# plurigrid/moose

Measured on AMD Instinct MI355X. Metric: replicated fixed(14,23) matmul elems/sec, higher is better.
Workload: dtype fixed(14,23) over Z_2^128 (exact multi-modular int8-MFMA GEMM)

## Files before the change

csrc/gemm_crt.hip:

```cpp
#include <hip/hip_runtime.h>

#include <algorithm>
#include <cmath>
#include <cstdint>
#include <cstdlib>
#include <cstring>
#include <mutex>

#include "hip_attr.h"
#include "moosex.h"
#include "prf_dev.h"
#include "rss_fused.h"

void mx_ws_note(int dev, int64_t want, bool ok);
bool mx_ws_malloc(void** p, int64_t bytes);
void mx_ws_shared_note(void);

namespace {

using u64 = uint64_t;
using u128 = unsigned __int128;
typedef int v4i __attribute__((ext_vector_type(4)));
typedef int v16i __attribute__((ext_vector_type(16)));

// ... 88 lines not shown
    for (int j = 0; j < n; ++j)
      if (j != i) {
        W *= (u128)kModuli[j];
        rest = (int)((int64_t)rest * kModuli[j] % p);
      }
    const int inv = modinv(rest, p);
    for (int k = 0; k < 8; ++k) t.rc.W[i][k] = (uint16_t)(W >> (16 * k));
    t.rc.rcp[i] = 1.0f / (float)p;
    t.ep.p[i] = p;
    t.ep.pf[i] = (float)p;
    t.ep.rcp[i] = 1.0f / (float)p;
    t.ep.t16[i] = (int)((1 << 16) % p);
    t.pa.p[i] = t.pb.p[i] = p;
    t.pa.rcp[i] = t.pb.rcp[i] = 1.0f / (float)p;
    int pw = 1 % p;
    for (int j = 0; j < nbytes; ++j) {
      const int wb = pw, wa = (int)((int64_t)pw * inv % p);
      t.pb.w[i][j / 4] |= (uint32_t)wb << (8 * (j % 4));
      t.pa.w[i][j / 4] |= (uint32_t)wa << (8 * (j % 4));
      pw = pw * 256 % p;
    }
    const int negb = (p - pw) % p;
    t.pb.neg[i] = (uint32_t)negb;
    t.pa.neg[i] = (uint32_t)((int64_t)negb * inv % p);
    if (i == 0) {
      t.pa.mul0 = (uint32_t)inv;
      t.pb.mul0 = 1;
    }
  }
  for (int k = 0; k < 8; ++k) t.rc.Mw[k] = (uint16_t)(Mw >> (16 * k));
  std::memset(&t.r4, 0, sizeof t.r4);
  t.r4.groups = (n + 3) / 4;
  for (int i = 0; i < n; ++i) {
    u128 W = 0;
    for (int k = 0; k < 8; ++k) W |= (u128)t.rc.W[i][k] << (16 * k);
    int carry = 0;
    for (int d = 0; d < nbytes; ++d) {
      int b = (int)((W >> (8 * d)) & 0xff) + carry;
      carry = b >= 128;
      b -= 256 * carry;
      t.r4.wd[i / 4][d] |= (uint32_t)(uint8_t)(int8_t)b << (8 * (i % 4));
    }
    int R = (int)std::lround(16777216.0 / kModuli[i]);
    for (int d = 0; d < 3; ++d) {
      int b = (R & 0xff);
      R >>= 8;
      if (b >= 128) {
        b -= 256;
        R += 1;
      }
      t.r4.rd[i / 4][d] |= (uint32_t)(uint8_t)(int8_t)b << (8 * (i % 4));
    }
  }
  (void)wbits;
}

const Tables& tables_for(int words, int n) {
  static std::mutex mu;
  static Tables cache[3][kMaxMod + 1];
  std::lock_guard<std::mutex> lk(mu);
  Tables& t = cache[words][n];
  if (t.n != n || t.words != words) build_tables(words, n, t);
  return t;
}

__device__ __forceinline__ uint32_t pack4(int a, int b, int c, int d) {
  const uint32_t lo = __builtin_amdgcn_perm((uint32_t)b, (uint32_t)a, 0x0c0c0400u);
  const uint32_t hi = __builtin_amdgcn_perm((uint32_t)d, (uint32_t)c, 0x0c0c0400u);
  return __builtin_amdgcn_perm(hi, lo, 0x05040100u);
}

template <class T>
struct Words;
template <>
struct Words<u64> {
  static constexpr int N = 2;
};
template <>
struct Words<u128> {
  static constexpr int N = 4;
};

template <int NW>
__device__ __forceinline__ int residue(const uint32_t (&x)[NW], const uint32_t (&w)[4],
                                       uint32_t neg, float p, float rcp) {
  uint32_t s = (x[NW - 1] >> 31) * neg;
#pragma unroll
  for (int q = 0; q < NW; ++q) s = __builtin_amdgcn_udot4(x[q], w[q], s, false);
  const float fs = (float)s;
  const float qt = __builtin_rintf(fs * rcp);
  return (int)__builtin_fmaf(-qt, p, fs);
}

typedef float f2 __attribute__((ext_vector_type(2)));
template <int NW>
__device__ __forceinline__ void residue2(const uint32_t (&xa)[NW], const uint32_t (&xb)[NW],
                                         const uint32_t (&w)[4], uint32_t neg, float p,
                                         float rcp, int& ra, int& rb) {
  uint32_t sa = 0, sb = 0;
#pragma unroll
  for (int q = 0; q < NW; ++q) {
    sa = __builtin_amdgcn_udot4(xa[q], w[q], sa, false);
    sb = __builtin_amdgcn_udot4(xb[q], w[q], sb, false);
  }
  const f2 sg = {(float)(xa[NW - 1] >> 31), (float)(xb[NW - 1] >> 31)};
  const float nf = (float)neg;
  const f2 fs = __builtin_elementwise_fma(sg, (f2){nf, nf}, (f2){(float)sa, (float)sb});
  f2 qt = fs * (f2){rcp, rcp};
  qt.x = __builtin_rintf(qt.x);
  qt.y = __builtin_rintf(qt.y);
  const f2 r = __builtin_elementwise_fma(-qt, (f2){p, p}, fs);
  ra = (int)r.x;
  rb = (int)r.y;
}

struct PrepSrcs {
  int n = 0;
  int mode[6];
  const void* x0[6];
  const void* x1[6];
  int64_t dual[6];
};

template <class T, bool TRANS, int ROWS, bool PK = true>
__global__ void __launch_bounds__(256)
    k_crt_prep(const T* __restrict__ X0, const T* __restrict__ X1, int64_t R, int64_t K,
               int64_t xs, int mode_all, int8_t* __restrict__ out, int64_t tiles, int64_t nkb,
               int64_t nkb_s, const PrepTab tab, const PrepSrcs src) {
  constexpr int NW = Words<T>::N;
  const int64_t total = tiles * nkb * (ROWS * 4);
  const int64_t b = blockIdx.y;
  const int mode = src.n > 0 ? src.mode[b] : mode_all;
  const T* x0 = src.n > 0 ? (const T*)src.x0[b] : X0 + b * xs;
  const T* x1 = src.n > 0 ? (const T*)src.x1[b] : (mode ? X1 + b * xs : x0);
  const int n = tab.n;
  const int64_t plane = tiles * nkb_s * (int64_t)(ROWS * BK);
  int8_t* ob = out + b * n * plane;
  for (int64_t g = blockIdx.x * (int64_t)blockDim.x + threadIdx.x; g < total;
       g += (int64_t)gridDim.x * blockDim.x) {
    const int c = (int)(g & 3);
    const int r = (int)((g >> 2) & (ROWS - 1));
    const int64_t q = g / (ROWS * 4);
    const int64_t kb = q % nkb, t = q / nkb;
    const int64_t row = t * ROWS + r;
    const int64_t k0 = kb * BK + c * 16;
    uint32_t v[16][NW];
#pragma unroll
    for (int j = 0; j < 16; ++j) {
      const int64_t k = k0 + j;
      T e = 0;
      if (row < R) {
        if (!TRANS) {
          if (k < K) e = mode == 2 ? (T)(x0[row * K + k] + x1[row * K + k]) : x0[row * K + k];
          else if (mode == 1 && k < 2 * K) e = x1[row * K + (k - K)];
        } else {
          if (k < K)
            e = (mode & 1) ? (T)(x0[k * R + row] + x1[k * R + row]) : x0[k * R + row];
          else if (mode == 1 && k < 2 * K) e = x0[(k - K) * R + row];
          else if (mode == 2 && k < 2 * K) e = x1[(k - K) * R + row];
        }
      }
#pragma unroll
      for (int w = 0; w < NW; ++w) v[j][w] = (uint32_t)(e >> (32 * w));
    }
    const int64_t boff = (t * nkb_s + kb) * (int64_t)(ROWS * BK) + img_off(r, c);
    auto emit = [&](int8_t* base) __attribute__((always_inline)) {
    {
      int rr[16];
#pragma unroll
      for (int j = 0; j < 16; ++j) rr[j] = (int)(v[j][0] * tab.mul0);
      v4i o;
#pragma unroll
      for (int u = 0; u < 4; ++u) o[u] = (int)pack4(rr[4 * u], rr[4 * u + 1], rr[4 * u + 2], rr[4 * u + 3]);
      *(v4i*)base = o;
    }
    for (int i = 1; i < n; ++i) {
      const uint32_t w[4] = {tab.w[i][0], tab.w[i][1], tab.w[i][2], tab.w[i][3]};
      const uint32_t neg = tab.neg[i];
      const float p = (float)tab.p[i], rcp = tab.rcp[i];
      int rr[16];
      if constexpr (PK) {
#pragma unroll
        for (int j = 0; j < 16; j += 2)
          residue2<NW>(v[j], v[j + 1], w, neg, p, rcp, rr[j], rr[j + 1]);
      } else {
#pragma unroll
        for (int j = 0; j < 16; ++j) rr[j] = residue<NW>(v[j], w, neg, p, rcp);
      }
      v4i o;
#pragma unroll
      for (int u = 0; u < 4; ++u) o[u] = (int)pack4(rr[4 * u], rr[4 * u + 1], rr[4 * u + 2], rr[4 * u + 3]);
      *(v4i*)(base + i * plane) = o;
    }
    };
    emit(ob + boff);
    if (src.n > 0 && src.dual[b]) {
#pragma unroll
      for (int j = 0; j < 16; ++j) {
        const int64_t k = k0 + j;
        if (row < R && k < K) {
          T e = 0;
#pragma unroll
          for (int w = 0; w < NW; ++w) e |= (T)v[j][w] << (32 * w);
          e += TRANS ? x1[k * R + row] : x1[row * K + k];
#pragma unroll
          for (int w = 0; w < NW; ++w) v[j][w] = (uint32_t)(e >> (32 * w));
        }
      }
      emit(ob + src.dual[b] + boff);
    }
  }
}

struct ShareSrc {
  const void* x = nullptr;
  int kind = 0;
  int frac = 0;
  int j0 = 0;
  uint64_t nonce = 0;
  mxd::KeySrc key;
};
struct SrcPlan {
  const void* x;
  int kind, pad;
  double scale;
  uint64_t nonce;
  int ph[4];
  int64_t off[4];
};

template <bool TRANS, int ROWS, bool PK>
__global__ void __launch_bounds__(256)
    k_crt_prep_src(const SrcPlan s, const mxd::KeySrc keys, int64_t R, int64_t K,
                   int8_t* __restrict__ out, int64_t tiles, int64_t nkb, const PrepTab tab) {
  using T = u128;
  constexpr int NW = 4;
  __shared__ uint32_t rks[1][mxd::kKeyWords];
  __shared__ uint4 xch[4][4][64];
  mxd::stage_keys(rks, keys, 1);
  const int lane = threadIdx.x & 63;
  const int p = lane & 3;
  uint4(*xw)[64] = xch[threadIdx.x >> 6];
  const int n = tab.n;
  const int64_t plane = tiles * nkb * (int64_t)(ROWS * BK);
  const int64_t total = tiles * ROWS * nkb * 4;
  for (int64_t g = blockIdx.x * (int64_t)blockDim.x + threadIdx.x; g < total;
       g += (int64_t)gridDim.x * blockDim.x) {
    const int c = (int)((g >> 2) & 3);
    const int rlow = (int)((g >> 4) & 3);
    const int64_t rest = g >> 6;
    int64_t row, kb, i0, istep;
    if (!TRANS) {
      const int64_t q = rest / (ROWS / 4);
      kb = 4 * (q % (nkb / 4)) + p;
      row = (q / (nkb / 4)) * ROWS + (rest % (ROWS / 4)) * 4 + rlow;
      i0 = row * K + (kb - p) * BK + c * 16;
      istep = 1;
    } else {
      const int64_t q = rest >> 4;
      kb = q % nkb;
      row = (q / nkb) * 256 + 64 * p + (rest & 15) * 4 + rlow;
      i0 = (kb * BK + c * 16) * R + (row - 64 * p);
      istep = R;
    }
    const bool live = row < R;
    const int64_t t = row / ROWS;
    const int r = (int)(row % ROWS);
    uint32_t v[16][NW];
#pragma unroll
    for (int jj = 0; jj < 4; ++jj) {
      uint32_t w[16];
      mx::chacha_block(rks[0], s.nonce, mx::ks_block_of((uint64_t)(i0 + (4 * jj + p) * istep)), w);
#pragma unroll
      for (int q = 0; q < 4; ++q)
        xw[q][lane ^ q] = make_uint4(w[4 * q], w[4 * q + 1], w[4 * q + 2], w[4 * q + 3]);
      __builtin_amdgcn_fence(__ATOMIC_RELEASE, "wavefront");
      __builtin_amdgcn_wave_barrier();
      __builtin_amdgcn_fence(__ATOMIC_ACQUIRE, "wavefront");
#pragma unroll
      for (int u = 0; u < 4; ++u) {
        const uint4 e = xw[p][((lane & ~3) | u) ^ p];
        v[4 * jj + u][0] = live ? e.x : 0u;
        v[4 * jj + u][1] = live ? e.y : 0u;
        v[4 * jj + u][2] = live ? e.z : 0u;
        v[4 * jj + u][3] = live ? e.w : 0u;
      }
      __builtin_amdgcn_fence(__ATOMIC_RELEASE, "wavefront");
      __builtin_amdgcn_wave_barrier();
      __builtin_amdgcn_fence(__ATOMIC_ACQUIRE, "wavefront");
    }
    const int64_t boff = (t * nkb + kb) * (int64_t)(ROWS * BK) + img_off(r, c);
    auto emit = [&](int8_t* base) __attribute__((always_inline)) {
      {
        int rr[16];
#pragma unroll
        for (int j = 0; j < 16; ++j) rr[j] = (int)(v[j][0] * tab.mul0);
        v4i o;
#pragma unroll
        for (int u = 0; u < 4; ++u) o[u] = (int)pack4(rr[4 * u], rr[4 * u + 1], rr[4 * u + 2], rr[4 * u + 3]);
        *(v4i*)base = o;
      }
      for (int i = 1; i < n; ++i) {
        const uint32_t w[4] = {tab.w[i][0], tab.w[i][1], tab.w[i][2], tab.w[i][3]};
        const uint32_t neg = tab.neg[i];
        const float pf = (float)tab.p[i], rcp = tab.rcp[i];
        int rr[16];
        if constexpr (PK) {
#pragma unroll
          for (int j = 0; j < 16; j += 2)
            residue2<NW>(v[j], v[j + 1], w, neg, pf, rcp, rr[j], rr[j + 1]);
        } else {
#pragma unroll
          for (int j = 0; j < 16; ++j) rr[j] = residue<NW>(v[j], w, neg, pf, rcp);
        }
        v4i o;
#pragma unroll
        for (int u = 0; u < 4; ++u) o[u] = (int)pack4(rr[4 * u], rr[4 * u + 1], rr[4 * u + 2], rr[4 * u + 3]);
        *(v4i*)(base + i * plane) = o;
      }
    };
    auto step = [&](bool sum) __attribute__((always_inline)) {
#pragma unroll
      for (int j = 0; j < 16; ++j) {
        T h = 0;
#pragma unroll
        for (int w = 0; w < NW; ++w) h |= (T)v[j][w] << (32 * w);
        const T x = live ? mxf::share_plain<T>(s.kind, s.x, i0 + 64 * p + j * istep, s.scale) : (T)0;
        const T other = mxf::share_masked<T>(s.kind, x, h);
        h = sum ? (T)(h + other) : other;
#pragma unroll
        for (int w = 0; w < NW; ++w) v[j][w] = (uint32_t)(h >> (32 * w));
      }
    };
#pragma nounroll
    for (int ph = 0; ph < 4; ++ph) {
      if (s.ph[0] != ph && s.ph[1] != ph && s.ph[2] != ph && s.ph[3] != ph) continue;
      if (ph == 1) step(false);
      if (ph == 2) step(true);
      if (ph == 3) {
#pragma unroll
        for (int j = 0; j < 16; ++j)
#pragma unroll
          for (int w = 0; w < NW; ++w) v[j][w] = 0;
      }
#pragma nounroll
      for (int e = 0; e < 4; ++e)
        if (s.ph[e] == ph) emit(out + s.off[e] + boff);
    }
  }
}

template <class T>
__global__ void __launch_bounds__(256)
    k_add_pair(const T* __restrict__ a, const T* __restrict__ b, T* __restrict__ o, int64_t n) {
  for (int64_t i = blockIdx.x * (int64_t)blockDim.x + threadIdx.x; i < n;
       i += (int64_t)gridDim.x * blockDim.x)
    o[i] = a[i] + b[i];
}

__device__ inline int64_t xcd_remap(int64_t bid, int64_t nwg) {
  const int64_t q = nwg / 8, r = nwg % 8;
  const int64_t x = bid % 8;
  return (x < r ? x * (q + 1) : r * (q + 1) + (x - r) * q) + bid / 8;
}

constexpr int waitcnt_vm_lgkm0(int vm) { return (vm & 15) | ((vm >> 4) << 14) | (7 << 4); }

__device__ __forceinline__ int centered_mod(int acc, float pf, float rcp, int t16) {
  const int hi = acc >> 16, lo = acc & 0xffff;
  const int s = __mul24(hi, t16) + lo;
  const float fs = (float)s;
  const float qt = __builtin_rintf(fs * rcp);
  return (int)__builtin_fmaf(-qt, pf, fs);
}

template <int WR, int WC, int BN, int MINW>
__global__ void __launch_bounds__(64 * WR * WC, MINW)
    k_crt_gemm(const int8_t* __restrict__ RA, const int8_t* __restrict__ RB,
               int8_t* __restrict__ CR, int tiles_m, int tiles_n, int nkb, int gM,
               const EpiTab ep, int dma_mask, int bcast) {
  constexpr int NW = WR * WC;
  constexpr int MI = BM / WR / 32, NJ = BN / WC / 32;
  constexpr int kImgB = BN * BK;
  constexpr int kStageBytes = kImg + kImgB;
  constexpr int NPIECE = kStageBytes / 1024;
  constexpr int PPW = NPIECE / NW;
  static_assert(PPW * NW == NPIECE, "stage pieces must split evenly over the waves");
  extern __shared__ __attribute__((aligned(16))) int8_t smem[];
  const int ntiles = tiles_m * tiles_n;
  const int tid_flat = (int)xcd_remap(blockIdx.x, ntiles);
  const int group = tid_flat / (gM * tiles_n);
  const int first_m = group * gM;
  const int gm = tiles_m - first_m < gM ? tiles_m - first_m : gM;
  const int in_group = tid_flat % (gM * tiles_n);
  const int tm = first_m + in_group % gm, tn = in_group / gm;
  const int g = blockIdx.y;
  const int mi = g % ep.n;
  const int8_t* ga = RA + ((int64_t)((bcast & 1) ? mi : g) * tiles_m + tm) * nkb * (int64_t)kImg;
  const int8_t* gb = RB + ((int64_t)((bcast & 2) ? mi : g) * tiles_n + tn) * nkb * (int64_t)kImgB;

  const int lane = threadIdx.x & 63;
  const int wave = __builtin_amdgcn_readfirstlane(threadIdx.x >> 6);
  const int wr = wave / WC, wc = wave % WC;
  const int half = lane >> 5;
  const int sw = swz(lane >> 2);
  const int rowa = (wr * (BM / WR) + (lane & 31)) * BK;
  const int rowb = kImg + (wc * (BN / WC) + (lane & 31)) * BK;
  const int co0 = 16 * (half ^ sw), co1 = 16 * ((2 + half) ^ sw);

  const int8_t* srcs[PPW];
  int dsts[PPW], steps[PPW];
#pragma unroll
  for (int t = 0; t < PPW; ++t) {
    const int pc = wave + NW * t;
    const bool is_b = pc >= 16;
    const int pp = is_b ? pc - 16 : pc;
    srcs[t] = (is_b ? gb : ga) + pp * 1024 + lane * 16;
    dsts[t] = (is_b ? kImg : 0) + pp * 1024;
    steps[t] = is_b ? kImgB : kImg;
  }
  auto dma = [&](int kb, int t, int8_t* dst_stage) {
    if (!((dma_mask >> (wave + NW * t >= 16 ? 1 : 0)) & 1)) return;
    __builtin_amdgcn_global_load_lds((const void*)(srcs[t] + (int64_t)kb * steps[t]),
                                     (__attribute__((address_space(3))) void*)(dst_stage + dsts[t]),
                                     16, 0, 0);
  };

  v16i acc[MI][NJ];
#pragma unroll
  for (int i = 0; i < MI; ++i)
// ... 939 lines not shown
  launch_recon<T>(p, tb, 3, M, N, cr, C, 0, st);
  const hipError_t e = hipGetLastError();
  return e != hipSuccess ? -100 - (int)e : 0;
}

}

extern "C" {

int mx_gemm_asym(int words, int64_t M, int64_t N, int64_t K, const void* S0, const void* S1,
                 const void* T0, const void* T1, int rolled, void* C, void* stream) {
  if (M == 0 || N == 0) return 0;
  if (!rolled && (!S1 || !T1)) return -2;
  hipStream_t st = (hipStream_t)stream;
  if (words == 1)
    return run_crt_asym<u64>(M, N, K, (const u64*)S0, (const u64*)S1, (const u64*)T0,
                             (const u64*)T1, rolled, (u64*)C, st);
  if (words == 2)
    return run_crt_asym<u128>(M, N, K, (const u128*)S0, (const u128*)S1, (const u128*)T0,
                              (const u128*)T1, rolled, (u128*)C, st);
  return -2;
}

int mx_gemm_asym_src(int words, int64_t M, int64_t N, int64_t K, const void* S0, const void* T0,
                     const int64_t* xsrc, const int64_t* ysrc, void* C, void* stream) {
  if (M == 0 || N == 0) return 0;
  if (words != 2) return -7;
  if ((!xsrc && !S0) || (!ysrc && !T0)) return -2;
  ShareSrc sx, sy;
  auto fill = [](ShareSrc& s, const int64_t* a) {
    s.x = (const void*)(intptr_t)a[0];
    s.kind = (int)a[1];
    s.frac = (int)a[2];
    s.j0 = (int)a[3];
    const uint32_t* slot[1] = {(const uint32_t*)(intptr_t)a[4]};
    s.key = mxd::keysrc_slots(slot, 1);
    s.nonce = (uint64_t)a[5];
  };
  if (xsrc) fill(sx, xsrc);
  if (ysrc) fill(sy, ysrc);
  if ((xsrc && !sx.key.slot[0]) || (ysrc && !sy.key.slot[0])) return -2;
  return run_crt_asym<u128>(M, N, K, (const u128*)S0, nullptr, (const u128*)T0, nullptr, 1,
                            (u128*)C, (hipStream_t)stream, xsrc ? &sx : nullptr,
                            ysrc ? &sy : nullptr);
}

int mx_crt_moduli(int words, int64_t kprime) {
  if (words != 1 && words != 2) return -2;
  return moduli_needed(words, kprime);
}

int mx_crt_tables(int words, int n, int32_t* p_out, uint8_t* wa_out, uint8_t* wb_out,
                  int32_t* nega_out, int32_t* negb_out, uint16_t* W_out, uint16_t* Mw_out) {
  if ((words != 1 && words != 2) || n < 1 || n > kMaxMod) return -2;
  const Tables& t = tables_for(words, n);
  for (int i = 0; i < n; ++i) {
    p_out[i] = t.ep.p[i];
    for (int j = 0; j < 16; ++j) {
      wa_out[i * 16 + j] = (uint8_t)(t.pa.w[i][j / 4] >> (8 * (j % 4)));
      wb_out[i * 16 + j] = (uint8_t)(t.pb.w[i][j / 4] >> (8 * (j % 4)));
    }
    nega_out[i] = (int32_t)t.pa.neg[i];
    negb_out[i] = (int32_t)t.pb.neg[i];
    if (i == 0) {
      nega_out[0] = (int32_t)t.pa.mul0;
      negb_out[0] = 1;
    }
    for (int k = 0; k < 8; ++k) W_out[i * 8 + k] = t.rc.W[i][k];
  }
  for (int k = 0; k < 8; ++k) Mw_out[k] = t.rc.Mw[k];
  return 0;
}

int mx_crt_tables4(int words, int n, uint32_t* wd_out, uint32_t* rd_out) {
  if ((words != 1 && words != 2) || n < 1 || n > kMaxMod) return -2;
  const Tables& t = tables_for(words, n);
  for (int g = 0; g < t.r4.groups; ++g) {
    for (int d = 0; d < 16; ++d) wd_out[g * 16 + d] = t.r4.wd[g][d];
    for (int d = 0; d < 3; ++d) rd_out[g * 3 + d] = t.r4.rd[g][d];
  }
  return t.r4.groups;
}

int mxh_gemm_crt(int words, int64_t batch, int64_t M, int64_t N, int64_t K, const void* A0,
                 const void* A1, const void* B0, const void* B1, int mode, void* C,
                 int accumulate, void* stream) {
  hipStream_t st = (hipStream_t)stream;
  if (words == 1)
    return run_crt<u64>(batch, M, N, K, (const u64*)A0, (const u64*)A1, M * K, (const u64*)B0,
                        (const u64*)B1, K * N, nullptr, mode, (u64*)C, accumulate, st);
  if (words == 2)
    return run_crt<u128>(batch, M, N, K, (const u128*)A0, (const u128*)A1, M * K,
                         (const u128*)B0, (const u128*)B1, K * N, nullptr, mode, (u128*)C,
                         accumulate, st);
  return -2;
}

int mxh_gemm_crt_strided(int words, int64_t batch, int64_t M, int64_t N, int64_t K,
                         const void* A0, const void* A1, int64_t a_bstride, const void* B0,
                         const void* B1, int64_t b_bstride, int mode, void* C, int accumulate,
                         void* stream) {
  hipStream_t st = (hipStream_t)stream;
  if (words == 1)
    return run_crt<u64>(batch, M, N, K, (const u64*)A0, (const u64*)A1, a_bstride,
                        (const u64*)B0, (const u64*)B1, b_bstride, nullptr, mode, (u64*)C,
                        accumulate, st);
  if (words == 2)
    return run_crt<u128>(batch, M, N, K, (const u128*)A0, (const u128*)A1, a_bstride,
                         (const u128*)B0, (const u128*)B1, b_bstride, nullptr, mode, (u128*)C,
                         accumulate, st);
  return -2;
}

int mxh_crt_roll(int words, int64_t batch, int64_t M, int64_t N, int64_t K, const void* A0,
                 int64_t a_bstride, int64_t roll, const void* B0, const void* B1, const void* rb,
                 void* C, int accumulate, void* stream) {
  hipStream_t st = (hipStream_t)stream;
  const int64_t bs = K * N;
  if (words == 1)
    return run_crt<u64>(batch, M, N, K, (const u64*)A0, nullptr, a_bstride, (const u64*)B0,
                        (const u64*)B1, bs, (const int8_t*)rb, 1, (u64*)C, accumulate, st, roll);
  if (words == 2)
    return run_crt<u128>(batch, M, N, K, (const u128*)A0, nullptr, a_bstride, (const u128*)B0,
                         (const u128*)B1, bs, (const int8_t*)rb, 1, (u128*)C, accumulate, st,
                         roll);
  return -2;
}

int64_t mxh_crt_b_bytes(int words, int64_t batch, int64_t N, int64_t K, int mode) {
  if (words != 1 && words != 2) return 0;
  const CPlan p = make_cplan(words, batch, BM, N, K, mode);
  return p.n < 0 ? 0 : p.rb_bytes;
}

int mxh_crt_prep_b(int words, int64_t batch, int64_t K, int64_t N, const void* B0,
                   const void* B1, int mode, void* rb, void* stream) {
  const CPlan p = make_cplan(words, batch, BM, N, K, mode);
  if (p.n < 0) return -6;
  const Tables& tb = tables_for(words, p.n);
  hipStream_t st = (hipStream_t)stream;
  if (words == 1)
    launch_prep<u64>(p, tb, true, batch, N, K, K * N, (const u64*)B0, (const u64*)B1, mode,
                     (int8_t*)rb, st);
  else if (words == 2)
    launch_prep<u128>(p, tb, true, batch, N, K, K * N, (const u128*)B0, (const u128*)B1, mode,
                      (int8_t*)rb, st);
  else
    return -2;
  const hipError_t e = hipGetLastError();
  return e != hipSuccess ? -100 - (int)e : 0;
}

int mxh_crt_with_b(int words, int64_t batch, int64_t M, int64_t N, int64_t K, const void* A0,
                   const void* A1, int64_t a_bstride, int mode, const void* rb, void* C,
                   int accumulate, void* stream) {
  hipStream_t st = (hipStream_t)stream;
  if (words == 1)
    return run_crt<u64>(batch, M, N, K, (const u64*)A0, (const u64*)A1, a_bstride, nullptr,
                        nullptr, 0, (const int8_t*)rb, mode, (u64*)C, accumulate, st);
  if (words == 2)
    return run_crt<u128>(batch, M, N, K, (const u128*)A0, (const u128*)A1, a_bstride, nullptr,
                         nullptr, 0, (const int8_t*)rb, mode, (u128*)C, accumulate, st);
  return -2;
}

}
// ... 1 lines not shown
```

csrc/moosex.h:

```cpp
#pragma once
#include <stdint.h>

#ifdef __cplusplus
extern "C" {
#endif

enum mx_binop { MX_ADD = 0, MX_SUB = 1, MX_MUL = 2, MX_AND = 3, MX_OR = 4, MX_XOR = 5 };
enum mx_unop { MX_NEG = 0, MX_NOT = 1, MX_SHL = 2, MX_SHR = 3, MX_SAR = 4 };
enum mx_cmpop { MX_LT = 0, MX_GT = 1, MX_EQ = 2, MX_MSB = 3 };
enum mx_cross { MX_CROSS_ARITH = 0, MX_CROSS_BOOL = 1 };
enum mx_share_src { MX_SHARE_F64 = 2, MX_SHARE_MIRROR = 8 };

typedef struct {
  uint32_t rk[44];
} mx_aes_key;

int mx_version(void);
int mx_device_count(void);

int mx_ew_binary(int dev, int op, int words, const void* a, int64_t na, const void* b,
                 int64_t nb, void* out, int64_t n, void* stream);
int mx_ew_binary_slot(int dev, int op, int words, const void* a, const void* b, int64_t nb,
                      void* out, int64_t m, int nparties, int which, void* stream);
int mx_add_zs3(int dev, int words, const void* v, const void* r, void* out0, void* out1,
// ... 19 lines not shown
              int64_t w_slot_stride, int64_t N, int64_t C, int64_t H, int64_t W, int64_t mult,
              int64_t KH, int64_t KW, int64_t sh, int64_t sw, int64_t pt, int64_t pl,
              int64_t dh, int64_t dw, int64_t OH, int64_t OW, int nhwc, void* stream);
int mx_ew_binary_slot2(int dev, int op, int words, const void* a0, const void* a1,
                       const void* b, int64_t nb, void* out0, void* out1, int64_t m,
                       int nparties, int which0, int which1, void* stream);
int mx_mul_trunc3_kv(int dev, int words, const void* x0, const void* x1, const void* y0,
                     const void* y1, void* out0, void* out1, int64_t n, int64_t ostride,
                     const uint32_t* slots, uint64_t nmul, int m, const uint64_t* nonces,
                     const int64_t* views, void* stream);
int mx_mul_trunc3_open(int dev, int words, const void* x, int64_t xstride, double* out,
                       int64_t n, const uint32_t* slots, uint64_t nmul, int m,
                       const uint64_t* nonces, int frac, void* stream);
int mx_ew_add3(int dev, int words, const void* a, const void* b, const void* c, void* out,
               int64_t n, void* stream);
int mx_lincomb2(int dev, int words, int nin, const void* const* ins, const int64_t* coef,
                const void* b, int64_t nb, void* out0, void* out1, int64_t m, int nparties,
                int which0, int which1, void* stream);
int mx_sum_views2(int dev, int words, const void* base0, const void* base1, int64_t is0,
                  int64_t is1, int64_t ps0, int64_t ps1, int k, void* out0, void* out1, int64_t m,
                  int nparties, void* stream);
int mx_slot_place2(int dev, int words, const void* x0, const void* x1, void* out0, void* out1,
                   int64_t m, int nparties, int which0, int which1, void* stream);
int mx_ew_compare(int dev, int op, int words, const void* a, int64_t na, const void* b,
                  int64_t nb, uint8_t* out, int64_t n, void* stream);
int mx_bit_extract(int dev, int words, const void* a, uint8_t* out, int64_t n, int bit,
                   void* stream);
int mx_ring_inject(int dev, int words, const uint8_t* bits, void* out, int64_t n, int bit,
                   void* stream);
int mx_encode(int dev, int words, const double* x, void* out, int64_t n, int frac,
              void* stream);
int mx_addn_decode(int dev, int words, const void* a, const void* b, const void* c,
                   const void* d, double* out, int64_t n, int frac, void* stream);
int mx_decode(int dev, int words, const void* x, double* out, int64_t n, int frac,
              void* stream);
int mx_fill(int dev, int words, void* out, int64_t n, uint64_t lo, uint64_t hi, void* stream);
int mx_bit_planes(int dev, int words, const void* a, uint8_t* out, int64_t outer, int64_t inner,
                  int start, int count, void* stream);
int mx_weighted_sum(int dev, int words, const void* a, const void* w, void* out, int64_t outer,
                    int64_t k, int64_t inner, void* stream);
int mx_sum_axis(int dev, int words, const void* a, void* out, int64_t outer, int64_t red,
                int64_t inner, void* stream);
int mx_prg(int dev, const uint8_t* key16, uint64_t nonce, uint64_t ctr0, void* out,
           int64_t nbytes, void* stream);
int mx_derive_seed(const uint8_t* key16, const uint8_t* sync16, uint8_t* out16);
int mx_aes_encrypt_blocks(const uint8_t* key16, const uint8_t* in, uint8_t* out,
                          int64_t nblocks);
int mx_rss_cross(int dev, int kind, int words, const void* x0, const void* x1,
                 const void* y0, const void* y1, void* out, int64_t n, int nparties,
                 const uint8_t* keys16, uint64_t nonce, void* stream);
int mx_zero_share(int dev, int kind, int words, void* out, int64_t n, int nparties,
                  const uint8_t* keys16, uint64_t nonce, void* stream);
int mx_prf_expand(int dev, int words, void* out, int64_t n, int nkeys,
                  const uint8_t* keys16, uint64_t nonce, void* stream);
int mx_gemm(int dev, int words, int64_t batch, int64_t M, int64_t N, int64_t K,
            const void* A0, const void* A1, const void* B0, const void* B1, int mode,
            void* C, int accumulate, void* stream);
int64_t mx_gemm_workspace_bytes(int words, int64_t batch, int64_t M, int64_t N,
                                int64_t K, int mode);
int64_t mx_workspace_failed_bytes(void);
int64_t mx_workspace_held_bytes(void);
int64_t mx_workspace_shared_count(void);
int mx_gemm_ws(int words, int64_t batch, int64_t M, int64_t N, int64_t K, const void* A0,
               const void* A1, const void* B0, const void* B1, int mode, void* C,
               int accumulate, void* workspace, int64_t ws_bytes, void* stream);
int64_t mx_gemm_b_bytes(int words, int64_t batch, int64_t N, int64_t K, int mode);
int mx_gemm_prep_b(int words, int64_t batch, int64_t K, int64_t N, const void* B0,
                   const void* B1, int mode, void* lb, void* stream);
int mx_gemm_with_b(int words, int64_t batch, int64_t M, int64_t N, int64_t K, const void* A0,
                   const void* A1, int64_t a_bstride, int mode, const void* lb, void* C,
                   int accumulate, void* stream);
int mx_crt_tables4(int words, int n, uint32_t* wd_out, uint32_t* rd_out);
int mx_gemm_roll(int words, int64_t batch, int64_t M, int64_t N, int64_t K, const void* A0,
                 int64_t a_bstride, int64_t roll, const void* B0, const void* B1, const void* lb,
                 void* C, int accumulate, void* stream);
int mx_gemm_strided(int words, int64_t batch, int64_t M, int64_t N, int64_t K, const void* A0,
                    const void* A1, int64_t a_bstride, const void* B0, const void* B1,
                    int64_t b_bstride, int mode, void* C, int accumulate, void* stream);
void mx_set_gemm_impl(int impl);
void mx_set_gemm_crt(int mode);
int mx_crt_moduli(int words, int64_t kprime);
int mx_crt_tables(int words, int n, int32_t* p, uint8_t* wa, uint8_t* wb, int32_t* nega,
                  int32_t* negb, uint16_t* W, uint16_t* Mw);

int mx_trunc_pr3(int dev, int words, const void* s0, void* out0, void* out1, int64_t n, int m,
                 const uint8_t* k0, const uint8_t* k2, const uint64_t* nonces, void* stream);
int mx_share3(int dev, int kind, int words, const void* x, void* out0, void* out1, int64_t n,
              int j, const uint8_t* k_next, const uint8_t* k_all, uint64_t n1, uint64_t na,
              void* stream);

#define MX_KEY_SLOT_WORDS 48
void mx_key_slots(const uint8_t* keys16, int n, uint32_t* out);
int mx_rss_cross_k(int dev, int kind, int words, const void* x0, const void* x1,
                   const void* y0, const void* y1, void* out, int64_t n, int nparties,
                   const uint32_t* slots, int nslots, uint64_t nonce, void* stream);
int mx_rss_cross_kp(int dev, int kind, int words, const void* x0, const void* x1,
                    const void* y0, const void* y1, void* out, int64_t n, int nparties,
                    const uint32_t* const* slot_ptrs, uint64_t nonce, void* stream);
int mx_rss_mul3_kv(int dev, int kind, int words, const void* x0, const void* x1, const void* y0,
                   const void* y1, void* out0, void* out1, int64_t n, const uint32_t* slots,
                   uint64_t nonce, const int64_t* views, void* stream);
int mx_rss_mul3_k(int dev, int kind, int words, const void* x0, const void* x1, const void* y0,
                  const void* y1, void* out0, void* out1, int64_t n, const uint32_t* slots,
                  uint64_t nonce, void* stream);
int mx_ks_adder3_k(int dev, int words, const void* g0, const void* g1, const void* p0,
                   const void* p1, void* og0, void* og1, int64_t n, int nlev,
                   const uint32_t* slots, const uint64_t* nonces, void* stream);
int mx_ks_level3_k(int dev, int words, const void* g0, const void* g1, const void* p0,
                   const void* p1, void* og0, void* og1, void* op0, void* op1, int64_t n,
                   int d, int both, const uint32_t* slots, uint64_t nonce, void* stream);
int mx_ks_cross1(int dev, int words, const void* g0, const void* g1, const void* p0,
                 const void* p1, void* z, int64_t n, int d, int both, const uint8_t* keys16,
                 uint64_t nonce, void* stream);
int mx_ks_cross1_s(int dev, int words, const void* g0, const void* g1, const void* p0,
                   const void* p1, void* z, int64_t n, int d, int both,
                   const uint32_t* const* slots, uint64_t nonce, void* stream);
int mx_ks_cross1x_s(int dev, int words, const void* g0, const void* g1, const void* t0,
                    const void* t1, void* go0, void* go1, const void* p0, const void* p1,
                    void* z, int64_t n, int d, int both, const uint32_t* const* slots,
                    uint64_t nonce, void* stream);
int mx_ks_sum2(int dev, int words, const void* p0, const void* p1, const void* g0,
               const void* g1, const void* t0, const void* t1, void* o0, void* o1, int64_t n,
               void* stream);
int mx_prf_expand_k(int dev, int words, void* out, int64_t n, int nkeys, const uint32_t* slots,
                    uint64_t nonce, void* stream);
int mx_trunc_pr3_k(int dev, int words, const void* s0, void* out0, void* out1, int64_t n, int m,
                   const uint32_t* slot_k0, const uint32_t* slot_k2, const uint64_t* nonces,
                   void* stream);
int mx_trunc_pr3_ko(int dev, int words, const void* s0, void* out0, void* out1, int64_t n,
                    int m, const uint32_t* slot_k0, const uint32_t* slot_k2,
                    const uint64_t* nonces, int64_t ostride, void* stream);
int mx_trunc_pr3_kmo(int dev, int words, const void* s0, void* out0, void* out1, int64_t n,
                     int m, const uint32_t* slot_k0, const uint32_t* slot_k2,
                     const uint64_t* nonces, int64_t ostride, const uint64_t* cm, void* stream);
int mx_share3_k(int dev, int kind, int words, const void* x, void* out0, void* out1, int64_t n,
                int j, const uint32_t* slot_next, const uint32_t* slot_all, uint64_t n1,
                uint64_t na, void* stream);
int mx_ring_extend3_k(int dev, const void* s0, void* out0, void* out1, int64_t n,
                      const uint32_t* slot_k0, const uint32_t* slot_k2, const uint64_t* nonces,
                      void* stream);
int64_t mx_ring_extend3_lat_max(void);

int mx_trunc_party_r0(int dev, int words, int64_t n, int m, int ncomp, const int* roles,
                      const void* s0, const void* s1, void* msg, void* msg_rm, void* out0,
                      void* out1, const uint32_t* const* slots, const uint64_t* nonces,
                      void* stream);
int mx_trunc_party_r1(int dev, int words, int64_t n, int m, int ncomp, const int* roles,
                      const void* msg, const void* rmk, const void* rrt, const void* rrm,
                      void* w, void* out0, void* out1, const uint32_t* const* slots,
                      const uint64_t* nonces, void* stream);
int mx_ring_extend_party_r0(int dev, int64_t n, int ncomp, const int* roles, const void* s0,
                            const void* s1, void* msg, void* msg_R, void* msg_M, void* out0,
                            void* out1, const uint32_t* const* slots, const uint64_t* nonces,
                            void* stream);
int mx_ring_extend_party_r1(int dev, int64_t n, int ncomp, const int* roles, const void* msg,
                            const void* rmk, const void* rR, const void* rM, void* w, void* out0,
                            void* out1, const uint32_t* const* slots, const uint64_t* nonces,
                            void* stream);
int mx_share_party(int dev, int kind, int words, int64_t n, int ncomp, const int* rel,
                   const void* x, void* out0, void* out1, const uint32_t* const* slots,
                   uint64_t n1, uint64_t na, void* stream);
int mx_dot_tail_r0(int dev, int words, int64_t n, int m, int ncomp, const int* roles,
                   const void* const* cross, void* const* msg, void* const* msg_rt,
                   void* const* msg_rm, void* const* out0, void* const* out1,
                   const uint32_t* const* slots, const uint64_t* nonces, void* stream);
int mx_dot_tail_r1(int dev, int words, int64_t n, int m, int ncomp, const int* roles,
// ... 40 lines not shown
```

moose_amd/ops/native.py:

```python
from __future__ import annotations

import ctypes
import os
import threading

import torch

from moose_amd import errors
from moose_amd._native import build as _build

_LIB = None
_LOCK = threading.Lock()

c_i64 = ctypes.c_int64
c_int = ctypes.c_int
c_u64 = ctypes.c_uint64
c_vp = ctypes.c_void_p

_SIGS = {
    "mx_version": (c_int, []),
    "mx_device_count": (c_int, []),
    "mx_ew_binary": (c_int, [c_int, c_int, c_int, c_vp, c_i64, c_vp, c_i64, c_vp, c_i64, c_vp]),
    "mx_ew_unary": (c_int, [c_int, c_int, c_int, c_vp, c_vp, c_i64, c_i64, c_vp]),
    "mx_mul_add2": (c_int, [c_int, c_int, c_vp, c_vp, c_vp, c_vp, c_int, c_int, c_vp, c_vp,
# ... 122 lines not shown
        [c_int, c_int, c_vp, c_vp, c_vp, c_vp, c_vp, c_vp, c_i64, c_int, c_vp, c_vp, c_vp],
    ),
    "mxh_ks_adder3_sum": (
        c_int,
        [c_int, c_vp, c_vp, c_vp, c_vp, c_vp, c_vp, c_i64, c_int, c_vp, c_vp, c_vp, c_int],
    ),
    "mx_ks_level3_k": (
        c_int,
        [c_int, c_int, c_vp, c_vp, c_vp, c_vp, c_vp, c_vp, c_vp, c_vp, c_i64, c_int, c_int,
         c_vp, c_u64, c_vp],
    ),
    "mx_rss_cross_kp": (
        c_int,
        [c_int, c_int, c_int, c_vp, c_vp, c_vp, c_vp, c_vp, c_i64, c_int, c_vp, c_u64, c_vp],
    ),
    "mx_rss_mul3_kv": (
        c_int,
        [c_int, c_int, c_int, c_vp, c_vp, c_vp, c_vp, c_vp, c_vp, c_i64, c_vp, c_u64, c_vp, c_vp],
    ),
    "mx_rss_mul3_k": (
        c_int,
        [c_int, c_int, c_int, c_vp, c_vp, c_vp, c_vp, c_vp, c_vp, c_i64, c_vp, c_u64, c_vp],
    ),
    "mx_trunc_pr3_k": (
        c_int, [c_int, c_int, c_vp, c_vp, c_vp, c_i64, c_int, c_vp, c_vp, c_vp, c_vp],
    ),
    "mx_trunc_pr3_ko": (
        c_int, [c_int, c_int, c_vp, c_vp, c_vp, c_i64, c_int, c_vp, c_vp, c_vp, c_i64, c_vp],
    ),
    "mx_trunc_pr3_kmo": (
        c_int, [c_int, c_int, c_vp, c_vp, c_vp, c_i64, c_int, c_vp, c_vp, c_vp, c_i64, c_vp,
                c_vp],
    ),
    "mx_share3_k": (
        c_int,
        [c_int, c_int, c_int, c_vp, c_vp, c_vp, c_i64, c_int, c_vp, c_vp, c_u64, c_u64, c_vp],
    ),
    "mx_ring_extend3_k": (c_int, [c_int, c_vp, c_vp, c_vp, c_i64, c_vp, c_vp, c_vp, c_vp]),
    "mx_ring_extend3_lat_max": (c_i64, []),
    "mx_trunc_party_r0": (
        c_int,
        [c_int, c_int, c_i64, c_int, c_int, c_vp, c_vp, c_vp, c_vp, c_vp, c_vp, c_vp, c_vp,
         c_vp, c_vp],
    ),
    "mx_trunc_party_r1": (
        c_int,
        [c_int, c_int, c_i64, c_int, c_int, c_vp, c_vp, c_vp, c_vp, c_vp, c_vp, c_vp, c_vp,
         c_vp, c_vp, c_vp],
    ),
    "mx_ring_extend_party_r0": (
        c_int,
        [c_int, c_i64, c_int, c_vp, c_vp, c_vp, c_vp, c_vp, c_vp, c_vp, c_vp, c_vp, c_vp, c_vp],
    ),
    "mx_ring_extend_party_r1": (
        c_int,
        [c_int, c_i64, c_int, c_vp, c_vp, c_vp, c_vp, c_vp, c_vp, c_vp, c_vp, c_vp, c_vp, c_vp],
    ),
    "mx_dot_tail_r0": (
        c_int,
        [c_int, c_int, c_i64, c_int, c_int, c_vp, c_vp, c_vp, c_vp, c_vp, c_vp, c_vp, c_vp,
         c_vp, c_vp],
    ),
    "mx_dot_tail_r1": (
        c_int,
        [c_int, c_int, c_i64, c_int, c_int, c_vp, c_vp, c_vp, c_vp, c_vp, c_vp, c_vp, c_vp,
         c_vp, c_vp, c_vp, c_vp],
    ),
    "mx_dot_tail_r2": (c_int, [c_int, c_int, c_i64, c_int, c_vp, c_vp, c_vp, c_vp, c_vp]),
    "mx_share_party": (
        c_int,
        [c_int, c_int, c_int, c_i64, c_int, c_vp, c_vp, c_vp, c_vp, c_vp, c_u64, c_u64, c_vp],
    ),
    "mx_gemm_b_bytes": (c_i64, [c_int, c_i64, c_i64, c_i64, c_int]),
    "mx_gemm_prep_b": (c_int, [c_int, c_i64, c_i64, c_i64, c_vp, c_vp, c_int, c_vp, c_vp]),
    "mx_gemm_with_b": (
        c_int,
        [c_int, c_i64, c_i64, c_i64, c_i64, c_vp, c_vp, c_i64, c_int, c_vp, c_vp, c_int, c_vp],
    ),
    "mx_share3": (
        c_int,
        [c_int, c_int, c_int, c_vp, c_vp, c_vp, c_i64, c_int, c_vp, c_vp, c_u64, c_u64, c_vp],
    ),
    "mx_crt_tables4": (c_int, [c_int, c_int, c_vp, c_vp]),
    "mx_copy_channels": (c_int, [c_vp, c_vp, c_i64, c_int, c_vp]),
    "mx_stream_cumask": (c_int, [c_vp, c_int, c_vp]),
    "mx_stream_destroy": (c_int, [c_vp]),
    "mx_graph_compose": (c_int, [c_int, c_vp, c_vp, c_vp, c_vp, c_vp, c_vp, c_vp, c_vp, c_vp]),
    "mx_graph_compose_merged": (c_int, [c_int, c_vp, c_vp, c_vp, c_vp, c_vp, c_vp, c_vp, c_vp,
                                        c_vp]),
    "mx_graph_dot": (c_int, [c_vp, ctypes.c_char_p, ctypes.c_uint]),
    "mx_graph_launch": (c_int, [c_vp, c_vp]),
    "mx_enable_peer": (c_int, [c_int, c_int]),
    "mx_alloc_uncached": (c_int, [c_int, c_i64, c_vp]),
    "mx_free_uncached": (c_int, [c_int, c_vp]),
    "mx_graph_build_chain": (c_int, [c_int, c_vp, c_vp, c_vp, c_vp, c_vp, c_vp, c_vp, c_vp,
                                     c_vp]),
    "mx_jobs_r0": (c_int, [c_int, c_int, c_int, c_vp, c_vp, c_i64, c_int, c_int, c_int, c_int,
                           c_vp, c_vp, c_vp, c_vp, c_vp, c_vp]),
    "mx_jobs_r0p": (c_int, [c_int, c_int, c_int, c_vp, c_vp, c_i64, c_int, c_int, c_int, c_int,
                            c_vp, c_vp, c_vp, c_vp, c_vp, c_int, c_vp, c_vp, c_vp]),
    "mx_jobs_r1": (c_int, [c_int, c_int, c_int, c_vp, c_vp, c_i64, c_int, c_int, c_vp, c_vp, c_vp,
                           c_vp, c_vp, c_vp, c_vp, c_vp, c_vp]),
    "mx_jobs_r2": (c_int, [c_int, c_int, c_int, c_vp, c_vp, c_i64, c_int, c_vp, c_vp, c_vp]),
    "mx_bits_front": (c_int, [c_int, c_int, c_int, c_i64, c_vp, c_vp, c_vp, c_vp, c_vp, c_vp,
                              c_vp, c_vp, c_vp, c_vp]),
    "mx_wsum_pair": (c_int, [c_int, c_int, c_int, c_int, c_int, c_int, c_int, c_i64, c_i64,
                             c_vp, c_vp, c_vp, c_vp, c_vp, c_vp, c_vp, c_vp, c_vp, c_vp, c_vp,
                             c_vp, c_vp, c_vp]),
    "mx_bits_b2a": (c_int, [c_int, c_int, c_int, c_int, c_i64, c_int, c_int, c_int, c_int,
                            c_vp, c_vp, c_vp,
                            c_vp, c_vp, c_vp, c_vp, c_vp, c_vp, c_vp, c_vp, c_vp]),
    "mx_key_refresh": (c_int, [c_vp, c_int, c_vp, c_vp, c_vp]),
    "mx_copy_async": (c_int, [c_vp, c_vp, ctypes.c_int64, c_vp]),
    "mx_key_refresh_host": (None, [c_vp, c_u64, c_int, c_vp]),
    "mx_copy_many": (c_int, [c_vp, c_int, c_i64, c_vp]),
    "mx_graph_free": (c_int, [c_vp, c_vp]),
    "mx_gemm_asym": (
        c_int, [c_int, c_i64, c_i64, c_i64, c_vp, c_vp, c_vp, c_vp, c_int, c_vp, c_vp],
    ),
    "mx_gemm_asym_src": (
        c_int, [c_int, c_i64, c_i64, c_i64, c_vp, c_vp, c_vp, c_vp, c_vp, c_vp],
    ),
    "mx_gemm_roll": (
        c_int,
        [c_int, c_i64, c_i64, c_i64, c_i64, c_vp, c_i64, c_i64, c_vp, c_vp, c_vp, c_vp, c_int,
         c_vp],
    ),
}


class NativeError(errors.KernelError):
    pass


def lib():
    global _LIB
    if _LIB is not None:
        return _LIB
    with _LOCK:
        if _LIB is not None:
            return _LIB
        if _build.needs_build() and os.environ.get("MOOSEX_NO_BUILD") != "1":
            _build.build()
        path = os.environ.get("MOOSEX_LIB") or str(_build.LIB)
        try:
            handle = ctypes.CDLL(path, mode=ctypes.RTLD_GLOBAL)
        except OSError as e:
            raise NativeError(f"cannot load {path}: {e}") from e
        for name, (res, args) in _SIGS.items():
            fn = getattr(handle, name)
            fn.restype = res
            fn.argtypes = args
        _LIB = handle
        return _LIB


def loaded_path():
    return str(_build.LIB)


def check(rc, what):
    if rc != 0:
        if rc == -4:
            raise NativeError(workspace_error(what, _ws_failed_bytes(), _ws_held_bytes()))
        raise NativeError(f"{what} failed with code {rc}")

# ... 79 lines not shown
```

Before: 1.398 billion.

## Derive sum-share CRT residues from component residues with carry correction

The fused share-and-prep kernel used to walk up to four phases serially. Each phase recomputed a full multi-word residue reduction for every modulus, and each sum phase re-ran the 128-bit add. It now computes the residues of the random share and the masked share once, then derives the residue of their sum by adding the two and applying a carry-count (kappa) correction times the wrap constant. The f64 plaintext loads are batched up front. This saves dot4 reductions and loop overhead but keeps more live registers (rr, v, kf, xp), and a host-side mx_crt_combine test hook is added.

```diff
diff --git a/csrc/gemm_crt.hip b/csrc/gemm_crt.hip
--- a/csrc/gemm_crt.hip
+++ b/csrc/gemm_crt.hip
@@ -194,21 +194,26 @@
 };
 
 template <int NW>
-__device__ __forceinline__ int residue(const uint32_t (&x)[NW], const uint32_t (&w)[4],
-                                       uint32_t neg, float p, float rcp) {
+__device__ __forceinline__ float residue_f(const uint32_t (&x)[NW], const uint32_t (&w)[4],
+                                           uint32_t neg, float p, float rcp) {
   uint32_t s = (x[NW - 1] >> 31) * neg;
 #pragma unroll
   for (int q = 0; q < NW; ++q) s = __builtin_amdgcn_udot4(x[q], w[q], s, false);
   const float fs = (float)s;
   const float qt = __builtin_rintf(fs * rcp);
-  return (int)__builtin_fmaf(-qt, p, fs);
+  return __builtin_fmaf(-qt, p, fs);
+}
+template <int NW>
+__device__ __forceinline__ int residue(const uint32_t (&x)[NW], const uint32_t (&w)[4],
+                                       uint32_t neg, float p, float rcp) {
+  return (int)residue_f<NW>(x, w, neg, p, rcp);
 }
 
 typedef float f2 __attribute__((ext_vector_type(2)));
 template <int NW>
-__device__ __forceinline__ void residue2(const uint32_t (&xa)[NW], const uint32_t (&xb)[NW],
+__device__ __forceinline__ f2 residue2_f(const uint32_t (&xa)[NW], const uint32_t (&xb)[NW],
                                          const uint32_t (&w)[4], uint32_t neg, float p,
-                                         float rcp, int& ra, int& rb) {
+                                         float rcp) {
   uint32_t sa = 0, sb = 0;
 #pragma unroll
   for (int q = 0; q < NW; ++q) {
@@ -221,9 +226,38 @@
   f2 qt = fs * (f2){rcp, rcp};
   qt.x = __builtin_rintf(qt.x);
   qt.y = __builtin_rintf(qt.y);
-  const f2 r = __builtin_elementwise_fma(-qt, (f2){p, p}, fs);
+  return __builtin_elementwise_fma(-qt, (f2){p, p}, fs);
+}
+template <int NW>
+__device__ __forceinline__ void residue2(const uint32_t (&xa)[NW], const uint32_t (&xb)[NW],
+                                         const uint32_t (&w)[4], uint32_t neg, float p,
+                                         float rcp, int& ra, int& rb) {
+  const f2 r = residue2_f<NW>(xa, xb, w, neg, p, rcp);
   ra = (int)r.x;
   rb = (int)r.y;
+}
+
+__host__ __device__ inline int crt_sum_kappa(uint32_t ta, uint32_t tb, uint32_t ts) {
+  const uint32_t carry = ((ta & tb) | ((ta | tb) & ~ts)) >> 31;
+  return (int)(ta >> 31) + (int)(tb >> 31) - (int)carry - (int)(ts >> 31);
+}
+__host__ __device__ inline float crt_combine_f(float ra, float rb, float kappa, float neg,
+                                               float p, float rcp) {
+  const float fs = __builtin_fmaf(kappa, -neg, ra + rb);
+  const float qt = __builtin_rintf(fs * rcp);
+  return __builtin_fmaf(-qt, p, fs);
+}
+__host__ __device__ inline int crt_combine(int ra, int rb, int kappa, uint32_t neg, float p,
+                                           float rcp) {
+  return (int)crt_combine_f((float)ra, (float)rb, (float)kappa, (float)neg, p, rcp);
+}
+__host__ __device__ inline f2 crt_combine2(f2 ra, f2 rb, f2 kappa, float neg, float p,
+                                           float rcp) {
+  const f2 fs = __builtin_elementwise_fma(kappa, (f2){-neg, -neg}, ra + rb);
+  f2 qt = fs * (f2){rcp, rcp};
+  qt.x = __builtin_rintf(qt.x);
+  qt.y = __builtin_rintf(qt.y);
+  return __builtin_elementwise_fma(-qt, (f2){p, p}, fs);
 }
 
 struct PrepSrcs {
@@ -378,7 +412,7 @@
     const bool live = row < R;
     const int64_t t = row / ROWS;
     const int r = (int)(row % ROWS);
-    uint32_t v[16][NW];
+    uint32_t rr[16][NW], v[16][NW];
 #pragma unroll
     for (int jj = 0; jj < 4; ++jj) {
       uint32_t w[16];
@@ -392,72 +426,125 @@
 #pragma unroll
       for (int u = 0; u < 4; ++u) {
         const uint4 e = xw[p][((lane & ~3) | u) ^ p];
-        v[4 * jj + u][0] = live ? e.x : 0u;
-        v[4 * jj + u][1] = live ? e.y : 0u;
-        v[4 * jj + u][2] = live ? e.z : 0u;
-        v[4 * jj + u][3] = live ? e.w : 0u;
+        rr[4 * jj + u][0] = live ? e.x : 0u;
+        rr[4 * jj + u][1] = live ? e.y : 0u;
+        rr[4 * jj + u][2] = live ? e.z : 0u;
+        rr[4 * jj + u][3] = live ? e.w : 0u;
       }
       __builtin_amdgcn_fence(__ATOMIC_RELEASE, "wavefront");
       __builtin_amdgcn_wave_barrier();
       __builtin_amdgcn_fence(__ATOMIC_ACQUIRE, "wavefront");
     }
+    float kf[16];
+    T xp[16];
+    if (s.kind == MX_SHARE_F64) {
+      double d[16];
+#pragma unroll
+      for (int j = 0; j < 16; ++j)
+        d[j] = live ? ((const double*)s.x)[i0 + 64 * p + j * istep] : 0.0;
+#pragma unroll
+      for (int j = 0; j < 16; ++j) xp[j] = mxf::share_plain<T>(MX_SHARE_F64, d, j, s.scale);
+    } else {
+#pragma unroll
+      for (int j = 0; j < 16; ++j)
+        xp[j] = live ? mxf::share_plain<T>(s.kind, s.x, i0 + 64 * p + j * istep, s.scale) : (T)0;
+    }
+#pragma unroll
+    for (int j = 0; j < 16; ++j) {
+      T h = 0;
+#pragma unroll
+      for (int w = 0; w < NW; ++w) h |= (T)rr[j][w] << (32 * w);
+      const T x = xp[j];
+      const T other = mxf::share_masked<T>(s.kind, x, h);
+#pragma unroll
+      for (int w = 0; w < NW; ++w) v[j][w] = (uint32_t)(other >> (32 * w));
+      kf[j] = (float)crt_sum_kappa(rr[j][NW - 1], v[j][NW - 1],
+                                   (uint32_t)((T)(h + other) >> (32 * (NW - 1))));
+    }
     const int64_t boff = (t * nkb + kb) * (int64_t)(ROWS * BK) + img_off(r, c);
-    auto emit = [&](int8_t* base) __attribute__((always_inline)) {
-      {
-        int rr[16];
-#pragma unroll
-        for (int j = 0; j < 16; ++j) rr[j] = (int)(v[j][0] * tab.mul0);
-        v4i o;
-#pragma unroll
-        for (int u = 0; u < 4; ++u) o[u] = (int)pack4(rr[4 * u], rr[4 * u + 1], rr[4 * u + 2], rr[4 * u + 3]);
-        *(v4i*)base = o;
-      }
-      for (int i = 1; i < n; ++i) {
-        const uint32_t w[4] = {tab.w[i][0], tab.w[i][1], tab.w[i][2], tab.w[i][3]};
-        const uint32_t neg = tab.neg[i];
-        const float pf = (float)tab.p[i], rcp = tab.rcp[i];
-        int rr[16];
+    bool has[4];
+#pragma unroll
+    for (int ph = 0; ph < 4; ++ph)
+      has[ph] = s.ph[0] == ph || s.ph[1] == ph || s.ph[2] == ph || s.ph[3] == ph;
+    const bool do_r = has[0] || has[2], do_v = has[1] || has[2];
+    auto put = [&](int ph, int64_t ioff, const v4i o) __attribute__((always_inline)) {
+#pragma unroll
+      for (int e = 0; e < 4; ++e)
+        if (s.ph[e] == ph) *(v4i*)(out + s.off[e] + ioff + boff) = o;
+    };
+    auto pack16 = [](const int (&q)[16]) __attribute__((always_inline)) {
+      v4i o;
+#pragma unroll
+      for (int u = 0; u < 4; ++u) o[u] = (int)pack4(q[4 * u], q[4 * u + 1], q[4 * u + 2], q[4 * u + 3]);
+      return o;
+    };
+    const v4i zero = {0, 0, 0, 0};
+    {
+      int q[16];
+#pragma unroll
+      for (int j = 0; j < 16; ++j) q[j] = (int)(rr[j][0] * tab.mul0);
+      put(0, 0, pack16(q));
+#pragma unroll
+      for (int j = 0; j < 16; ++j) q[j] = (int)(v[j][0] * tab.mul0);
+      put(1, 0, pack16(q));
+#pragma unroll
+      for (int j = 0; j < 16; ++j) q[j] = (int)((rr[j][0] + v[j][0]) * tab.mul0);
+      put(2, 0, pack16(q));
+      put(3, 0, zero);
+    }
+    for (int i = 1; i < n; ++i) {
+      const uint32_t w[4] = {tab.w[i][0], tab.w[i][1], tab.w[i][2], tab.w[i][3]};
+      const uint32_t neg = tab.neg[i];
+      const float pf = (float)tab.p[i], rcp = tab.rcp[i];
+      const int64_t ioff = i * plane;
+      const float nf = (float)neg;
+      auto res4 = [&](const uint32_t (&x)[16][NW], int u, float (&f)[4])
+                      __attribute__((always_inline)) {
         if constexpr (PK) {
 #pragma unroll
-          for (int j = 0; j < 16; j += 2)
-            residue2<NW>(v[j], v[j + 1], w, neg, pf, rcp, rr[j], rr[j + 1]);
+          for (int j = 0; j < 4; j += 2) {
+            const f2 g = residue2_f<NW>(x[4 * u + j], x[4 * u + j + 1], w, neg, pf, rcp);
+            f[j] = g.x;
+            f[j + 1] = g.y;
+          }
         } else {
 #pragma unroll
-          for (int j = 0; j < 16; ++j) rr[j] = residue<NW>(v[j], w, neg, pf, rcp);
+          for (int j = 0; j < 4; ++j) f[j] = residue_f<NW>(x[4 * u + j], w, neg, pf, rcp);
         }
-        v4i o;
-#pragma unroll
-        for (int u = 0; u < 4; ++u) o[u] = (int)pack4(rr[4 * u], rr[4 * u + 1], rr[4 * u + 2], rr[4 * u + 3]);
-        *(v4i*)(base + i * plane) = o;
-      }
-    };
-    auto step = [&](bool sum) __attribute__((always_inline)) {
-#pragma unroll
-      for (int j = 0; j < 16; ++j) {
-        T h = 0;
-#pragma unroll
-        for (int w = 0; w < NW; ++w) h |= (T)v[j][w] << (32 * w);
-        const T x = live ? mxf::share_plain<T>(s.kind, s.x, i0 + 64 * p + j * istep, s.scale) : (T)0;
-        const T other = mxf::share_masked<T>(s.kind, x, h);
-        h = sum ? (T)(h + other) : other;
-#pragma unroll
-        for (int w = 0; w < NW; ++w) v[j][w] = (uint32_t)(h >> (32 * w));
-      }
-    };
-#pragma nounroll
-    for (int ph = 0; ph < 4; ++ph) {
-      if (s.ph[0] != ph && s.ph[1] != ph && s.ph[2] != ph && s.ph[3] != ph) continue;
-      if (ph == 1) step(false);
-      if (ph == 2) step(true);
-      if (ph == 3) {
-#pragma unroll
-        for (int j = 0; j < 16; ++j)
-#pragma unroll
-          for (int w = 0; w < NW; ++w) v[j][w] = 0;
-      }
-#pragma nounroll
-      for (int e = 0; e < 4; ++e)
-        if (s.ph[e] == ph) emit(out + s.off[e] + boff);
+      };
+      v4i o_r, o_v, o_s;
+#pragma unroll
+      for (int u = 0; u < 4; ++u) {
+        float fr[4], fv[4], fs[4];
+        if (do_r) {
+          res4(rr, u, fr);
+          o_r[u] = (int)pack4((int)fr[0], (int)fr[1], (int)fr[2], (int)fr[3]);
+        }
+        if (do_v) {
+          res4(v, u, fv);
+          o_v[u] = (int)pack4((int)fv[0], (int)fv[1], (int)fv[2], (int)fv[3]);
+        }
+        if (has[2]) {
+          if constexpr (PK) {
+#pragma unroll
+            for (int j = 0; j < 4; j += 2) {
+              const f2 g = crt_combine2((f2){fr[j], fr[j + 1]}, (f2){fv[j], fv[j + 1]},
+                                        (f2){kf[4 * u + j], kf[4 * u + j + 1]}, nf, pf, rcp);
+              fs[j] = g.x;
+              fs[j + 1] = g.y;
+            }
+          } else {
+#pragma unroll
+            for (int j = 0; j < 4; ++j)
+              fs[j] = crt_combine_f(fr[j], fv[j], kf[4 * u + j], nf, pf, rcp);
+          }
+          o_s[u] = (int)pack4((int)fs[0], (int)fs[1], (int)fs[2], (int)fs[3]);
+        }
+      }
+      put(0, ioff, o_r);
+      put(1, ioff, o_v);
+      put(2, ioff, o_s);
+      put(3, ioff, zero);
     }
   }
 }
@@ -1563,6 +1650,25 @@
   return t.r4.groups;
 }
 
+int mx_crt_combine(int words, int n, int side, int i, int64_t count, const int32_t* ra,
+                   const int32_t* rb, const int32_t* kappa, int8_t* out) {
+  if ((words != 1 && words != 2) || n < 1 || n > kMaxMod || i < 0 || i >= n || (side & ~1))
+    return -2;
+  const Tables& t = tables_for(words, n);
+  const PrepTab& tab = side ? t.pb : t.pa;
+  const float p = (float)tab.p[i], rcp = tab.rcp[i];
+  for (int64_t k = 0; k < count; ++k) {
+    if (side) {
+      out[k] = (int8_t)crt_combine(ra[k], rb[k], kappa[k], tab.neg[i], p, rcp);
+    } else {
+      const f2 f = crt_combine2((f2){(float)ra[k], 0.f}, (f2){(float)rb[k], 0.f},
+                                (f2){(float)kappa[k], 0.f}, (float)tab.neg[i], p, rcp);
+      out[k] = (int8_t)(int)f.x;
+    }
+  }
+  return 0;
+}
+
 int mxh_gemm_crt(int words, int64_t batch, int64_t M, int64_t N, int64_t K, const void* A0,
                  const void* A1, const void* B0, const void* B1, int mode, void* C,
                  int accumulate, void* stream) {
diff --git a/csrc/moosex.h b/csrc/moosex.h
--- a/csrc/moosex.h
+++ b/csrc/moosex.h
@@ -125,6 +125,8 @@
 int mx_crt_moduli(int words, int64_t kprime);
 int mx_crt_tables(int words, int n, int32_t* p, uint8_t* wa, uint8_t* wb, int32_t* nega,
                   int32_t* negb, uint16_t* W, uint16_t* Mw);
+int mx_crt_combine(int words, int n, int side, int i, int64_t count, const int32_t* ra,
+                   const int32_t* rb, const int32_t* kappa, int8_t* out);
 
 int mx_trunc_pr3(int dev, int words, const void* s0, void* out0, void* out1, int64_t n, int m,
                  const uint8_t* k0, const uint8_t* k2, const uint64_t* nonces, void* stream);
diff --git a/moose_amd/ops/native.py b/moose_amd/ops/native.py
--- a/moose_amd/ops/native.py
+++ b/moose_amd/ops/native.py
@@ -228,6 +228,7 @@
         [c_int, c_int, c_int, c_vp, c_vp, c_vp, c_i64, c_int, c_vp, c_vp, c_u64, c_u64, c_vp],
     ),
     "mx_crt_tables4": (c_int, [c_int, c_int, c_vp, c_vp]),
+    "mx_crt_combine": (c_int, [c_int, c_int, c_int, c_int, c_i64, c_vp, c_vp, c_vp, c_vp]),
     "mx_copy_channels": (c_int, [c_vp, c_vp, c_i64, c_int, c_vp]),
     "mx_stream_cumask": (c_int, [c_vp, c_int, c_vp]),
     "mx_stream_destroy": (c_int, [c_vp]),
```

Result: faster. 1.464 billion (median of 6 runs) (+4.7%).
